# NeLy-EPFL/flygym

Hardware: AMD Instinct MI355X
Metric: env-steps/sec (whole node), 4096 flies per GPU, flat terrain (higher is better)
Workload: dtype f32

## Files before the change

### flygym_amd/csrc/nmf_step.hip

```cpp
#include "nmf_device.h"
#include "nmf_step_lds.h"
#include "nmf_step_diag.h"
#include "nmf_step_kinematics.h"
#include "nmf_step_collision.h"
#include "nmf_step_aba.h"
#include "nmf_step_contact.h"
#include "nmf_dual.h"
#include "nmf_step_noslip.h"
#include "nmf_step_actuation.h"
#include "nmf_step_forward.h"
#include "nmf_step_io.h"
#include "nmf_tree.h"

namespace nmf {

template <class TP> constexpr int waves_per_simd() { return 2; }

template <class TP>
__device__ __forceinline__ void stage_launch_constants(FlyLds<TP>& s, const GModel& m) {
  if constexpr (!TP::kStar) { if (threadIdx.x == 0) { s.rt_nb = m.nb; s.rt_nv = m.nv; } __syncthreads(); }
  if constexpr (TP::kNFact > 1) {
    for (int b = threadIdx.x; b < TP::kTblB && b < m.nb; b += kWave) {
      s.t_body[b] = (unsigned char)m.tree_body[b < m.tree_lvl_start[m.tree_nlevel] ? b : 0];
      s.t_parent[b] = (unsigned char)(b ? m.body_parent[b] : 0);
      s.t_dofadr[b] = (unsigned char)m.body_dofadr[b]; s.t_dofnum[b] = (unsigned char)m.body_dofnum[b];
      s.t_cstart[b] = (unsigned char)m.tree_child_start[b]; s.t_ccount[b] = (unsigned char)m.tree_child_count[b];
    }
    for (int j = threadIdx.x; j < TP::kTblV && j < m.nv; j += kWave) s.t_dofbody[j] = (unsigned char)m.dof_body[j];
    if (threadIdx.x < 18) s.t_lvl[threadIdx.x] = (unsigned char)m.tree_lvl_start[threadIdx.x];
    if (threadIdx.x == 0) s.t_nlevel = (unsigned char)m.tree_nlevel;
    if constexpr (TP::kStar) {
      for (int i = threadIdx.x; i < kRestLevels * 16; i += kWave) (&s.t_pack[0][0][0])[i] = m.rest_fast ? m.rest_pack[i] : 0xffffffffu;
    }
    __syncthreads();
  }
  const int lane = threadIdx.x;
  for (int j = lane; j < s.nv(); j += kWave) {
    if constexpr (row_width_s<TP>() > 6) s.S[j][6] = 0.f;
    s.arm[j] = m.dof_armature[j];
    if constexpr (kHasCm3<TP>) { s.damp[j] = m.dof_damping[j]; s.dlt[j] = m.dof_armature[j] + m.timestep * m.dof_damping[j]; }
  }
  if (lane < 6) {
    const KLane K = k_lane(lane, make_frame(v3(m.plane[0], m.plane[1], m.plane[2])));
    float* q = s.k_tab[lane];
#pragma unroll
    for (int i = 0; i < 3; ++i) { q[i] = K.dA[i]; q[3 + i] = K.dB[i]; q[6 + i] = K.dO[i]; }
    q[9] = __int_as_float(K.ia); q[10] = __int_as_float(K.ib);
    int words[3];
    inertia_map_pack(lane, words);
    q[11] = __int_as_float(words[0]); q[12] = __int_as_float(words[1]); q[13] = __int_as_float(words[2]);
    if constexpr (kHasIsym<TP>) {
#pragma unroll
      for (int c = 0; c < 6; c++) {
        const int i = lane < c ? lane : c, jx = lane < c ? c : lane;
        q[14 + c] = __int_as_float(i * 6 - i * (i - 1) / 2 + (jx - i));
      }
    }
  }
  if constexpr (kHasIsym<TP>) if (lane == 0) {
    const Frame fr = make_frame(v3(m.plane[0], m.plane[1], m.plane[2]));
    st3(&s.frame9[0], fr.n); st3(&s.frame9[3], fr.t1); st3(&s.frame9[6], fr.t2);
    HotModel& h = s.hot;
    h.dof_axis = m.dof_axis; h.body_pos = m.body_pos; h.body_quat = m.body_quat; h.geom_p0 = m.geom_p0; h.geom_p1 = m.geom_p1;
    h.geom_radius = m.geom_radius; h.geom_bsphere = m.geom_bsphere; h.hull_vert = m.hull_vert; h.pair_margin = m.pair_margin;
    h.geom_body = m.geom_body; h.geom_type = m.geom_type; h.geom_hulladr = m.geom_hulladr; h.geom_hullnum = m.geom_hullnum;
#pragma unroll
    for (int i = 0; i < 4; ++i) h.plane[i] = m.plane[i];
#pragma unroll
    for (int i = 0; i < 5; ++i) h.terrain[i] = m.terrain[i];
    h.hull_skin = m.hull_skin; h.terrain_type = m.terrain_type; h.ng = m.ng; h.sem_max_hull_contacts = m.sem_max_hull_contacts;
    h.terrain_walls = m.sem_terrain_walls;
  }
  if constexpr (kHasIsym<TP>) for (int i = lane; i < 3 * s.nv(); i += kWave) (&s.axis[0][0])[i] = m.dof_axis[i];
}

template <class TP>
__global__ void __launch_bounds__(kWave) nmf_reset_kernel(const DevModel* __restrict__ mp, DevState st, const unsigned char* __restrict__ reset_mask) {
  __shared__ FlyLds<TP> s;
  const GModel& m = *(const GModel*)mp;
  const int lane = threadIdx.x, w = (int)blockIdx.x;
  if (w >= st.n_worlds || (reset_mask && !reset_mask[w])) return;
  stage_launch_constants(s, m);
  for (int i = lane; i < s.nq(); i += kWave) s.qpos[i] = m.key_qpos[i];
  for (int i = lane; i < s.nv(); i += kWave) { s.qvel[i] = 0.f; s.qacc[i] = 0.f; }
  for (int i = lane; i < m.nu; i += kWave) { s.ctrl[i] = m.key_ctrl[i]; st.actuator_force[(size_t)w * m.nu + i] = 0.f; st.act[(size_t)w * m.nu + i] = 0.f; }
  for (int i = lane; i < 96; i += kWave) st.sensordata[(size_t)w * 96 + i] = 0.f;
  if (lane == 0) { s.ncon = 0; s.iters = 0; s.overflow = 0; s.solve_resid = 0.f; }
  WSYNC();
  stage_kinematics(s, m, lane);
  write_poses(s, m, st, w, lane);
  write_outputs(s, m, st, w, lane, 0.f, true);
  if (lane < 16) st.stats_sum[16 * (size_t)w + lane] = 0u;
  if (lane < kActHistWords) st.act_hist[(size_t)w * kActHistWords + lane] = 0u;
  if (lane < kMaxCon) st.contact_geom[(size_t)w * kMaxCon + lane] = -1.f;
}

template <class TP, bool WELD>
__global__ void __launch_bounds__(kWave) __attribute__((amdgpu_waves_per_eu(waves_per_simd<TP>(), waves_per_simd<TP>()))) nmf_step_kernel(const DevModel* __restrict__ mp, DevState st, ReplayArgs rp, int n_steps) {
  __shared__ FlyLds<TP> s;
  const GModel& m = *(const GModel*)mp;
  const unsigned long long probe_c0 = __builtin_amdgcn_s_memtime(), probe_r0 = __builtin_amdgcn_s_memrealtime();
  TRACE_DECL();
  const int lane = threadIdx.x;
  const bool chunked = st.sched_mode == 1;
  unsigned int t_first = 0;
  if (chunked && lane == 0) t_first = atomicAdd(&st.csched->ticket, 1u);
  stage_launch_constants(s, m);
  if constexpr (kDualGlob<TP>) { if (lane == 0) s.dual_glob[0] = st.dual_scratch + (size_t)blockIdx.x * kDualScratchFloats; }
  if constexpr (kEulerFused<TP>) {
    if (lane == 0) {
      const unsigned long long p = (unsigned long long)(st.dual_scratch + (size_t)blockIdx.x * euler_scratch_floats<TP>());
      s.euler_fac[0] = (unsigned int)p; s.euler_fac[1] = (unsigned int)(p >> 32);
    }
  }
  unsigned int t_next = (unsigned int)__builtin_amdgcn_readfirstlane((int)t_first);
  STAGE_INIT();
  const int n_chunks = chunked ? st.n_chunks : 1;
  const unsigned int epoch = chunked ? (unsigned int)__builtin_amdgcn_readfirstlane((int)st.csched->epoch) : 0u;
  for (;;) {
    int slot = (int)blockIdx.x, chunk = 0, step0 = 0, step1 = n_steps;
    if (chunked) {
      const unsigned int t = t_next;
      if (t >= (unsigned int)st.n_worlds * (unsigned int)n_chunks) {
        if (lane == 0 && atomicAdd(&st.csched->exited, 1u) == gridDim.x - 1u) {
          st.csched->ticket = 0u; st.csched->exited = 0u; st.csched->epoch = epoch + 1u;
        }
        break;
      }
      chunk = (int)(t / (unsigned int)st.n_worlds); slot = (int)(t % (unsigned int)st.n_worlds);
      step0 = st.chunk_start[chunk]; step1 = st.chunk_start[chunk + 1];
    } else if (slot >= st.n_worlds) return;
    const int w = __builtin_amdgcn_readfirstlane(st.order ? st.order[slot] : slot);
    TRACE_SUB(2);
    const unsigned long long t_begin = __builtin_amdgcn_s_memtime();
    if (st.sched && lane == 0) atomicMin(&st.sched->t_first, (unsigned long long)__builtin_amdgcn_s_memrealtime());
    float time;
    unsigned int carry = 0u;
    unsigned int sum_con = 0u, sum_it = 0u, sum_of = 0u;
    unsigned int sum_dual = 0u, sum_kkt = 0u;
    {
      const float* tab = rp.table ? rp.table + (size_t)w * rp.table_steps * rp.n_act : nullptr;
      const int ln = opaque(lane);
      const int my_ctrl = tab && lane < rp.n_act ? rp.act_ids[ln] : -1;
      CtrlPrefetch pf;
      pf.mine = my_ctrl >= 0; pf.next_row = nullptr;
      pf.value = my_ctrl >= 0 ? tab[(size_t)((rp.start + step0) % rp.table_steps) * rp.n_act + lane] : 0.f;
      if (chunk > 0) {
        const unsigned int want = (unsigned int)__builtin_amdgcn_readfirstlane((int)(epoch * 32u + (unsigned int)chunk));
        const unsigned long long* hb = st.handoff + (size_t)w * st.handoff_stride;
        const int nq = s.nq(), nv = s.nv();
        for (;;) {
          bool ok = true;
          for (int i = ln; i < nq; i += kWave) s.qpos[i] = ld_tagged(&hb[i], want, ok);
          for (int i = ln; i < nv; i += kWave) { s.qvel[i] = ld_tagged(&hb[nq + i], want, ok); s.qacc[i] = ld_tagged(&hb[nq + nv + i], want, ok); }
          for (int i = ln; i < m.nu; i += kWave) s.ctrl[i] = ld_tagged(&hb[nq + 2 * nv + i], want, ok);
          carry = lane < 6 ? ld_tagged_u(&hb[nq + 2 * nv + m.nu + ln], want, ok) : 0u;
          if constexpr (kDual<TP>) { const unsigned int hw = lane < hist_words<TP>(m) ? ld_tagged_u(&hb[nq + 2 * nv + m.nu + 6 + ln], want, ok) : 0u; if (lane < kHistLds<TP>) s.act_hist[lane] = hw; }
          if (!__any(!ok)) break;
          __builtin_amdgcn_s_sleep(8);
        }
        time = __uint_as_float((unsigned int)__builtin_amdgcn_readlane((int)carry, 0));
      } else {
        for (int i = ln; i < s.nq(); i += kWave) s.qpos[i] = ld_state(&st.qpos[(size_t)w * s.nq() + i]);
        for (int i = ln; i < s.nv(); i += kWave) {
          s.qvel[i] = ld_state(&st.qvel[(size_t)w * s.nv() + i]);
          s.qacc[i] = ld_state(&st.qacc_ws[(size_t)w * s.nv() + i]);
        }
        for (int i = ln; i < m.nu; i += kWave) s.ctrl[i] = ld_state(&st.ctrl[(size_t)w * m.nu + i]);
        if constexpr (kDual<TP>) { if (lane < kHistLds<TP>) s.act_hist[lane] = st.act_hist[(size_t)w * kActHistWords + ln]; }
        time = ld_state(&st.time[w]);
      }
      WSYNC();
      TRACE_GAP_END();
      for (int step = step0; step < step1; ++step) {
        if (tab) {
          if (my_ctrl >= 0) s.ctrl[my_ctrl] = pf.value;
          const float* src = tab + (size_t)((rp.start + step) % rp.table_steps) * rp.n_act;
          for (int a = opaque(lane) + kWave; a < rp.n_act; a += kWave) s.ctrl[rp.act_ids[a]] = src[a];
          pf.next_row = step + 1 < step1 ? tab + (size_t)((rp.start + step + 1) % rp.table_steps) * rp.n_act : nullptr;
          WSYNC();
        }
        STAGE(0);
        float* rec = nullptr;
        if (st.obs_every > 0 && (step + 1) % st.obs_every == 0)
          rec = st.ring + ((size_t)((step + 1) / st.obs_every - 1) * (size_t)st.n_worlds + (size_t)w) * (size_t)st.ring_stride;
        const bool wrenches = physics_forward<TP, WELD>(s, m, lane, st, w, step == n_steps - 1, rec, pf STAGE_PASS);
        physics_integrate<TP, WELD>(s, m, lane, wrenches STAGE_PASS);
        if (rec) {
          const int nj = st.ring_nj;
          for (int i = opaque(lane); i < nj; i += kWave) { rec[i] = s.qpos[7 + i]; rec[nj + i] = s.qvel[6 + i]; }
        }
        STAGE(15);
        time += m.timestep;
        const unsigned int rep = (unsigned int)__builtin_amdgcn_readfirstlane(s.iters);
        sum_con += (unsigned int)s.ncon; sum_it += rep & 0xffu; sum_of += (unsigned int)s.overflow;
        sum_dual += (rep >> 8) & 1u; sum_kkt += (rep >> 9) & 1u;
        if (rep & (0xffcu << 8)) {
          const int xl = opaque(lane) - 6;
          if (xl >= 2 && xl < kExitKinds && ((rep >> (8 + xl)) & 1u)) add_count(&st.stats_sum[16 * (size_t)w + 4 + xl], 1u);
        }
      }
    }
    TRACE_BUSY_END();
    TRACE_SUB_RESET();
    unsigned int t_new = 0;
    if (chunked && lane == 0) t_new = atomicAdd(&st.csched->ticket, 1u);
    {
      const unsigned int own = lane == 1 ? (unsigned int)(step1 - step0) : lane == 2 ? sum_con : lane == 3 ? sum_it : sum_of;
      const float cyc = (float)(__builtin_amdgcn_s_memtime() - t_begin);
      if (lane >= 1 && lane <= 4) carry += own;
      if (lane == 5) carry = __float_as_uint(__uint_as_float(carry) + cyc);
      const bool final = step1 == n_steps;
      if (lane == 6 || lane == 7) add_count(&st.stats_sum[16 * (size_t)w + opaque(lane) - 2], lane == 6 ? sum_dual : sum_kkt);
      write_outputs(s, m, st, w, lane, time, final, epoch * 32u + (unsigned int)(chunk + 1), carry);
      if (final) {
        if (lane >= 1 && lane <= 4) add_count(&st.stats_sum[16 * (size_t)w + opaque(lane) - 1], carry);
        if (lane == 5) st_state(&st.cost[w], __uint_as_float(carry));
      }
      if (st.sched && lane == 0) atomicMax(&st.sched->t_last, (unsigned long long)__builtin_amdgcn_s_memrealtime());
    }
    if (!chunked) break;
    TRACE_SUB(0);
    t_next = (unsigned int)__builtin_amdgcn_readfirstlane((int)t_new);
    TRACE_SUB(1);
    WSYNC();
  }
  TRACE_FLUSH();
  if (blockIdx.x == 0 && lane == 0 && st.clock_probe) {
    atomicAdd(&st.clock_probe[0], __builtin_amdgcn_s_memtime() - probe_c0);
    atomicAdd(&st.clock_probe[1], __builtin_amdgcn_s_memrealtime() - probe_r0);
  }
  STAGE(16);
  STAGE_FLUSH();
}

#define NMF_INSTANTIATE(k, TP, ...) NMF_IF_TOPO_##k(                                                      \
  template __global__ void nmf_step_kernel<TP, false>(const DevModel*, DevState, ReplayArgs, int);        \
  template __global__ void nmf_step_kernel<TP, true>(const DevModel*, DevState, ReplayArgs, int);         \
  template __global__ void nmf_step_kernel<Terrain<TP>, false>(const DevModel*, DevState, ReplayArgs, int);)
NMF_FAMILIES(NMF_INSTANTIATE)
#undef NMF_INSTANTIATE

}
```

### flygym_amd/csrc/nmf_step_collision.h

```cpp
#pragma once
#include "nmf_device.h"

namespace nmf {

__device__ __forceinline__ float terrain_kind(int kind, float p0, float p1, float p2, float x, float y) {
  if (kind == 1) { const float period = p0 + p1; const float u = x - floorf(x / period) * period; return u < p0 ? 0.f : -p2; }
  if (kind == 2) { const float i = floorf(x / p0), j = floorf(y / p0); const float sum = i + j;
                   const float par = sum - 2.f * floorf(sum / 2.f); return par != 0.f ? p1 : 0.f; }
  return 0.f;
}
__device__ __forceinline__ float terrain_height(int terrain_type, const float* p, float x, float y) {
  if (terrain_type == 3) {
    const float st = floorf(x / p[3]); const float k = st - 3.f * floorf(st / 3.f);
    return k == 1.f ? terrain_kind(1, 1.0f, p[1], p[2], x, y) : (k == 2.f ? terrain_kind(2, p[0], 0.35f, 0.f, x, y) : 0.f);
  }
  return terrain_kind(terrain_type, p[0], p[1], p[2], x, y);
}

constexpr float kFar = 1e30f;
constexpr float kProbeEps = 1e-4f;
constexpr float kOneCell = 0.02f;
__device__ __forceinline__ float terrain_cell_kind(int kind, float p0, float p1, float p2, float x, float y, float* b) {
  b[0] = -kFar; b[1] = kFar; b[2] = -kFar; b[3] = kFar;
  if (kind == 1) {
    const float period = p0 + p1; const float k = floorf(x / period); const float u = x - k * period;
    if (u < p0) { b[0] = k * period; b[1] = k * period + p0; return 0.f; }
    b[0] = k * period + p0; b[1] = (k + 1.f) * period; return -p2;
  }
  if (kind == 2) {
    const float i = floorf(x / p0), j = floorf(y / p0);
    b[0] = i * p0; b[1] = (i + 1.f) * p0; b[2] = j * p0; b[3] = (j + 1.f) * p0;
    const float sum = i + j; const float par = sum - 2.f * floorf(sum / 2.f);
    return par != 0.f ? p1 : 0.f;
  }
  return 0.f;
}
__device__ __forceinline__ float terrain_cell(int terrain_type, const float* p, float x, float y, float* b) {
  if (terrain_type == 3) {
    const float st = floorf(x / p[3]); const float k = st - 3.f * floorf(st / 3.f);
    const float h = k == 1.f ? terrain_cell_kind(1, 1.0f, p[1], p[2], x, y, b) : (k == 2.f ? terrain_cell_kind(2, p[0], 0.35f, 0.f, x, y, b)
                                                                                            : terrain_cell_kind(0, 0.f, 0.f, 0.f, x, y, b));
    const float lo = st * p[3], hi = (st + 1.f) * p[3];
    if (b[0] < lo) b[0] = lo;
    if (b[1] > hi) b[1] = hi;
    return h;
  }
  return terrain_cell_kind(terrain_type, p[0], p[1], p[2], x, y, b);
}
__device__ __forceinline__ void terrain_probe(int terrain_type, const float* p, bool walls, float x, float y, float zc, float rho,
                                              float reach, float& dtop, float& dwall, int& wall) {
  float b[4];
  const float h0 = terrain_cell(terrain_type, p, x, y, b);
  const float zb = zc - rho;
  dtop = zb - h0; dwall = kFar; wall = 0;
  if (!walls) return;
  const float delta[4] = {b[1] - x, x - b[0], b[3] - y, y - b[2]};
  if (zb >= h0 && fminf(fminf(delta[0], delta[1]), fminf(delta[2], delta[3])) - rho > reach) return;
  const float pen0 = h0 - zb;
  float he[4];
#pragma unroll
  for (int e = 0; e < 4; ++e) {
    he[e] = h0;
    if (delta[e] < kFar && (delta[e] - rho <= reach || (zb < h0 && delta[e] + rho < pen0)))
      he[e] = e == 0 ? terrain_height(terrain_type, p, b[1] + kProbeEps, y) : e == 1 ? terrain_height(terrain_type, p, b[0] - kProbeEps, y)
            : e == 2 ? terrain_height(terrain_type, p, x, b[3] + kProbeEps) : terrain_height(terrain_type, p, x, b[2] - kProbeEps);
  }
  float edge_top = kFar;
#pragma unroll
  for (int e = 0; e < 4; ++e) {
    if (!(delta[e] - rho <= reach && he[e] > zb)) continue;
    if (zc - he[e] > delta[e]) edge_top = fminf(edge_top, zb - he[e]);
    else if (delta[e] - rho < dwall) { dwall = delta[e] - rho; wall = (e ^ 1) + 1; }
  }
  if (zb < h0) {
    float pen = h0 - zb; int code = 0;
#pragma unroll
    for (int e = 0; e < 4; ++e)
      if (delta[e] < kFar && he[e] <= zb && delta[e] + rho < pen) { pen = delta[e] + rho; code = e + 1; }
    if (code) { dtop = kFar; if (-pen < dwall) { dwall = -pen; wall = code; } }
  }
  dtop = fminf(dtop, edge_top);
}

struct CollisionScratch {
  float r[kMaxCon][3], dist[kMaxCon];
  int info[kMaxCon];
};

__device__ __forceinline__ float readlane_f(float v, int lane) {
  return __builtin_bit_cast(float, __builtin_amdgcn_readlane(__builtin_bit_cast(int, v), lane));
}

template <class TP, bool ROUGH>
__device__ __noinline__ void stage_collision(FlyLds<TP>& s, const GModel& m, int lane) {
  static_assert(sizeof(CollisionScratch) <= sizeof(float) * TP::NB * 12, "collision scratch does not fit T..W");
  CollisionScratch& X = *reinterpret_cast<CollisionScratch*>(&s.T[0][0]);
  constexpr bool kSlotInTW = sizeof(CollisionScratch) + 2 * kWave * sizeof(int) <= sizeof(float) * TP::NB * 12;
  static_assert(kSlotInTW || 3 * (TP::NB - 1) + 2 * kWave <= 7 * kMaxCon, "slot table (128 geoms) does not fit");
  int* geom_slot0 = kSlotInTW ? reinterpret_cast<int*>(&s.T[0][0]) + sizeof(CollisionScratch) / sizeof(int)
                              : reinterpret_cast<int*>(&s.c_w[0][0]) + 3 * (TP::NB - 1);
  constexpr int kTwUsed = (int)sizeof(CollisionScratch) + (kSlotInTW ? 2 * kWave * (int)sizeof(int) : 0);
  constexpr int kCandRoom = ((int)sizeof(float) * TP::NB * 12 - kTwUsed) / 8;
  constexpr int kCand = kCandRoom > kWave ? kWave : kCandRoom;
  constexpr bool kListed = ROUGH && kCand >= 8;
  int* cand_idx = reinterpret_cast<int*>(&s.T[0][0]) + kTwUsed / 4;
  float* cand_d = reinterpret_cast<float*>(cand_idx + (kCand > 0 ? kCand : 0));
  const HotModel hm = hot_model(s, m);
  const int ng = hm.ng, terrain_type = hm.terrain_type, max_hull_contacts = hm.sem_max_hull_contacts;
  const bool walls = hm.terrain_walls != 0;
  const float hull_skin = hm.hull_skin, terrain_top = hm.terrain[4];
  const float tpar[4] = {hm.terrain[0], hm.terrain[1], hm.terrain[2], hm.terrain[3]};
  const gptr<int> geom_body = G(hm.geom_body), geom_type = G(hm.geom_type), geom_hulladr = G(hm.geom_hulladr),
                  geom_hullnum = G(hm.geom_hullnum);
  const gptr<float> pair_margin = G(hm.pair_margin), geom_bsphere = G(hm.geom_bsphere), geom_radius = G(hm.geom_radius),
                    geom_p0 = G(hm.geom_p0), geom_p1 = G(hm.geom_p1), hull_vert = G(hm.hull_vert);
  const V3 n = ld3(hm.plane);
  const float pd = hm.plane[3];
  const V3 o = ld3(s.xpos()[0]);
  constexpr bool rough = ROUGH;
  SUB_T0();
  int nh = 0, slot_base = 0;
  for (int g0 = 0; g0 < ng; g0 += kWave) {
  const int gi = g0 + lane;
  int g_body = 0, g_type = -1, g_hadr = 0, g_hnum = 0, cnt = 0;
  float g_margin = 0.f, cd0 = 0.f, cd1 = 0.f;
  V3 cp0 = v3(0, 0, 0), cp1 = v3(0, 0, 0);
  float cdw0 = 0.f, cdw1 = 0.f; V3 cpw0 = v3(0, 0, 0), cpw1 = v3(0, 0, 0); int cfid = 0, cntw = 0;
  bool near = false;
  bool one_cell = false; float g_ttop = 0.f;
  if (gi < ng) {
    g_body = geom_body[gi]; g_type = geom_type[gi]; g_margin = pair_margin[gi];
    g_hadr = geom_hulladr[gi]; g_hnum = geom_hullnum[gi];
    const V3 bs = ld3(geom_bsphere + 4 * gi);
    const float bs_r = geom_bsphere[4 * gi + 3], rad = geom_radius[gi];
    const V3 l0 = ld3(geom_p0 + 3 * gi), l1 = ld3(geom_p1 + 3 * gi);
    const float* R = s.xmat()[g_body];
    const V3 xp = ld3(s.xpos()[g_body]);
    V3 cw = mat_vec(R, bs);
    float dc = dot(n, cw) + dot(n, xp) - pd;
    float ttop = terrain_top;
    const V3 p0 = mat_vec(R, l0) + xp, p1 = mat_vec(R, l1) + xp;
    if (rough && dc - bs_r - terrain_top <= g_margin) {
      const float cx = cw.x + xp.x, cy = cw.y + xp.y, fr = bs_r + g_margin, fc = rad + g_margin;
      const float fx0 = fmaxf(cx - fr, fminf(p0.x, p1.x) - fc), fx1 = fminf(cx + fr, fmaxf(p0.x, p1.x) + fc);
      const float fy0 = fmaxf(cy - fr, fminf(p0.y, p1.y) - fc), fy1 = fminf(cy + fr, fmaxf(p0.y, p1.y) + fc);
      const float mx = 0.5f * (fx0 + fx1), my = 0.5f * (fy0 + fy1);
      float cb[4];
      ttop = terrain_cell(terrain_type, tpar, mx, my, cb);
      const float clear = fminf(fminf(cb[1] - fx1, fx0 - cb[0]), fminf(cb[3] - fy1, fy0 - cb[2]));
      one_cell = clear > kOneCell;
      if (!(clear > 0.f)) {
        if (terrain_type >= 2 && tpar[0] < 0.5f * (fy1 - fy0)) ttop = terrain_top;
        else {
          float xs = fx0;
          bool open = true;
#pragma unroll 1
          for (int k = 0; k < 8 && open; ++k) {
            float wb[4];
            ttop = fmaxf(ttop, terrain_cell(terrain_type, tpar, xs, my, wb));
            ttop = fmaxf(ttop, fmaxf(terrain_height(terrain_type, tpar, xs, fy0), terrain_height(terrain_type, tpar, xs, fy1)));
            open = wb[1] <= fx1;
            xs = wb[1] + kProbeEps;
          }
          if (open) ttop = terrain_top;
        }
      }
      g_ttop = ttop;
    }
    near = dc - bs_r - ttop <= g_margin;
    const float z0 = dot(n, p0) - pd, z1 = dot(n, p1) - pd;
    float d0 = z0 - rad, d1 = z1 - rad;
    if (g_type == GEOM_HULL) {
      const V3 ax = p1 - p0;
      const float ca = dot(n, ax);
      const float sn = sqrtf(fmaxf(0.f, 1.f - ca * ca / fmaxf(dot(ax, ax), 1e-12f)) + 4e-6f);
      near = near && fminf(z0, z1) - rad * fminf(sn, 1.f) - ttop <= g_margin;
    } else if (rough) near = near && fminf(d0, d1) - ttop <= g_margin;
    if (near && g_type == GEOM_CAPSULE) {
      float dw0 = kFar, dw1 = kFar; int w0 = 0, w1 = 0;
      if (rough) {
        if (one_cell && fminf(d0, d1) - g_ttop >= -kOneCell) { d0 -= g_ttop; d1 -= g_ttop; }
        else {
          terrain_probe(terrain_type, tpar, walls, p0.x, p0.y, z0, rad, g_margin, d0, dw0, w0);
          terrain_probe(terrain_type, tpar, walls, p1.x, p1.y, z1, rad, g_margin, d1, dw1, w1);
        }
      }
      const V3 q0 = ((p0 - rad * n) - (0.5f * d0) * n) - o, q1 = ((p1 - rad * n) - (0.5f * d1) * n) - o;
      if (d0 <= g_margin) { cd0 = d0; cp0 = q0; cnt = 1; }
      if (d1 <= g_margin) { if (cnt) { cd1 = d1; cp1 = q1; } else { cd0 = d1; cp0 = q1; } cnt++; }
      if (rough) {
        if (w0 && dw0 <= g_margin) { const V3 nw = contact_frame(w0, Frame{n, n, n}).n; cdw0 = dw0; cpw0 = ((p0 - rad * nw) - (0.5f * dw0) * nw) - o; cfid = w0; cntw = 1; }
        if (w1 && dw1 <= g_margin) { const V3 nw = contact_frame(w1, Frame{n, n, n}).n; const V3 q = ((p1 - rad * nw) - (0.5f * dw1) * nw) - o;
                                     if (cntw) { cdw1 = dw1; cpw1 = q; cfid |= w1 << 3; } else { cdw0 = dw1; cpw0 = q; cfid = w1; } cntw++; }
        cnt += cntw;
      }
    }
  }
  SUB(21);
  unsigned long long hmask = __ballot(near && g_type == GEOM_HULL);
  const unsigned long long one_mask = __ballot(one_cell);
  SUB_COUNT(24, __popcll(hmask));
  while (hmask) {
    SUBH_T0();
    const int g = __ffsll((long long)hmask) - 1;
    hmask &= hmask - 1;
    const int b = __builtin_amdgcn_readlane(g_body, g);
    const float margin = readlane_f(g_margin, g);
    const gptr<float> V = hull_vert + 3 * __builtin_amdgcn_readlane(g_hadr, g);
    const int nvv = __builtin_amdgcn_readlane(g_hnum, g);
    const float* R = s.xmat()[b];
    const V3 xp = ld3(s.xpos()[b]);
    const V3 nb = matT_vec(R, n);
    const float c0 = dot(n, xp) - pd;
    float pdw = kFar; int pw_code = 0;
    bool one = rough && ((one_mask >> g) & 1ull);
    const float h_top = rough ? readlane_f(g_ttop, g) : 0.f;
    auto vdist = [&](V3 v) {
      float di = dot(nb, v) + c0;
      if (rough) {
        pw_code = 0;
        if (one || di - h_top > margin) di = di - h_top;
        else { const V3 pw = mat_vec(R, v) + xp; terrain_probe(terrain_type, tpar, walls, pw.x, pw.y, di, 0.f, margin, di, pdw, pw_code); }
      }
      return di;
    };
    SUBH(28);
    float best = INFINITY; int bi = 0x7fffffff;
    float bestw = INFINITY; int biw = 0x7fffffff;
    int ncand = 0;
    for (;;) {
    best = INFINITY; bi = 0x7fffffff; ncand = 0;
    for (int base = lane; base < nvv + lane; base += 4 * kWave) {
      V3 hv[4];
#pragma unroll
      for (int k = 0; k < 4; ++k) { const int i = base + k * kWave; hv[k] = ld3(V + 3 * (i < nvv ? i : nvv - 1)); }
#pragma unroll
      for (int k = 0; k < 4; ++k) {
        const int i = base + k * kWave;
        bool c = false; float di = 0.f;
        if (i < nvv) {
          di = vdist(hv[k]);
          if (di < best) { best = di; bi = i; }
          if (rough && pw_code && pdw < bestw) { bestw = pdw; biw = i * 8 + pw_code; }
          c = di <= margin;
        }
        if constexpr (kListed) {
          const unsigned long long cm = __ballot(c);
          const int pos = ncand + __popcll(cm & ((1ull << lane) - 1ull));
          if (c && pos < kCand) { cand_idx[pos] = i; cand_d[pos] = di; }
          ncand += __popcll(cm);
        }
      }
    }
    wave_argmin(best, bi);
    if (rough && one && !(best >= -kOneCell)) { one = false; continue; }
    break;
    }
    const float dmin = best; const int ia = bi;
    bool face = false;
    if (rough && walls) { wave_argmin(bestw, biw); face = bestw <= margin; }
    SUBH(29); SUB_COUNT(32, one ? 1 : 0); SUB_COUNT(33, nvv);
    if (!(dmin <= margin) && !face) { SUB_COUNT(25, 1); SUB_COUNT(26, (unsigned long long)(fminf(dmin, 1.f) * 1e6f)); continue; }
    SUB_COUNT(27, 1);
    int nsel = 0;
    int s1 = -1, s2 = -1, s3 = -1;
    [[maybe_unused]] int listed_dbg = 0;
    if (dmin <= margin) {
    nsel = 1;
    const float thr = fminf(dmin + hull_skin, margin);
    const V3 va = ld3(V + 3 * ia);
    bool listed = false;
    if constexpr (kListed) listed = ncand <= kCand;
    listed_dbg = listed ? 1 : 0;
    if (listed) {
      if constexpr (kListed) {
        WSYNC();
        const bool have = lane < ncand;
        const int ci = have ? cand_idx[lane] : 0;
        const bool ok = have && !(cand_d[have ? lane : 0] > thr);
        const V3 vi = ld3(V + 3 * ci);
        auto pick = [&](int idx) {
          const int wl = __ffsll((long long)__ballot(ok && ci == idx)) - 1;
          return v3(readlane_f(vi.x, wl), readlane_f(vi.y, wl), readlane_f(vi.z, wl));
        };
        { const V3 e = vi - va; best = ok ? dot(e, e) : -INFINITY; bi = ok ? ci : 0x7fffffff; }
        wave_argmax(best, bi);
        if (best > 1e-10f) {
          s1 = bi; nsel = 2;
          const V3 ab = pick(bi) - va;
          const float lab2 = dot(ab, ab);
          { const V3 cr = cross(vi - va, ab); best = ok ? dot(cr, cr) : -INFINITY; bi = ok ? ci : 0x7fffffff; }
          wave_argmax(best, bi);
          if (best > 1e-10f * lab2) {
            s2 = bi; nsel = 3;
            const float side = dot(cross(pick(bi) - va, ab), nb);
            const float sg = side > 0.f ? -1.f : 1.f;
            best = ok ? sg * dot(cross(vi - va, ab), nb) : -INFINITY; bi = ok ? ci : 0x7fffffff;
            wave_argmax(best, bi);
            if (best > sqrtf(1e-10f * lab2)) { s3 = bi; nsel = 4; }
          }
        }
        WSYNC();
      }
    } else {
    best = -INFINITY; bi = 0x7fffffff;
    for (int i = lane; i < nvv; i += kWave) {
      V3 vi = ld3(V + 3 * i);
      float di = vdist(vi);
      if (di > thr) continue;
      V3 e = vi - va; float sc = dot(e, e);
      if (sc > best) { best = sc; bi = i; }
    }
    wave_argmax(best, bi);
    if (best > 1e-10f) {
      s1 = bi; nsel = 2;
      const V3 ab = ld3(V + 3 * bi) - va;
      const float lab2 = dot(ab, ab);
      best = -INFINITY; bi = 0x7fffffff;
      for (int i = lane; i < nvv; i += kWave) {
        V3 vi = ld3(V + 3 * i);
        float di = vdist(vi);
        if (di > thr) continue;
        V3 cr = cross(vi - va, ab); float sc = dot(cr, cr);
        if (sc > best) { best = sc; bi = i; }
      }
      wave_argmax(best, bi);
      if (best > 1e-10f * lab2) {
        s2 = bi; nsel = 3;
        const float side = dot(cross(ld3(V + 3 * bi) - va, ab), nb);
        const float sg = side > 0.f ? -1.f : 1.f;
        best = -INFINITY; bi = 0x7fffffff;
        for (int i = lane; i < nvv; i += kWave) {
          V3 vi = ld3(V + 3 * i);
          float di = vdist(vi);
          if (di > thr) continue;
          float sc = sg * dot(cross(vi - va, ab), nb);
          if (sc > best) { best = sc; bi = i; }
        }
        wave_argmax(best, bi);
        if (best > sqrtf(1e-10f * lab2)) { s3 = bi; nsel = 4; }
      }
    }
    }
    nsel = nsel < max_hull_contacts ? nsel : max_hull_contacts;
    }
    SUBH(30); SUB_COUNT(34, listed_dbg);
    if (lane < nsel && nh + lane < kMaxCon) {
      const int vi = lane == 0 ? ia : lane == 1 ? s1 : lane == 2 ? s2 : s3;
      const V3 v = ld3(V + 3 * vi);
      float dist = lane == 0 ? dmin : vdist(v);
      if (rough && lane != 0 && !(dist <= margin)) dist = fminf(dmin + hull_skin, margin);
      const V3 pw = mat_vec(R, v) + xp;
      X.info[nh + lane] = (g0 + g) | (lane << 8) | (b << 12);
      X.dist[nh + lane] = dist;
      st3(X.r[nh + lane], (pw - (0.5f * dist) * n) - o);
    }
    if (face && lane == nsel && nh + lane < kMaxCon) {
      const int code = biw & 7;
      const V3 nw = contact_frame(code, Frame{n, n, n}).n;
      const V3 pw = mat_vec(R, ld3(V + 3 * (biw >> 3))) + xp;
      X.info[nh + lane] = (g0 + g) | (lane << 8) | (b << 12) | (code << 20);
      X.dist[nh + lane] = bestw;
      st3(X.r[nh + lane], (pw - (0.5f * bestw) * nw) - o);
    }
    nsel += face ? 1 : 0;
    if (lane == g) cnt = nsel;
    nh += nsel;
    SUBH(31);
  }
  SUB(22);
  const unsigned long long b0 = __ballot(cnt & 1), b1 = __ballot(cnt & 2), b2 = __ballot(cnt & 4);
  const unsigned long long lt = (1ull << lane) - 1ull;
  const int slot0 = __popcll(b0 & lt) + 2 * __popcll(b1 & lt) + 4 * __popcll(b2 & lt);
  const int sl = slot_base + slot0;
  geom_slot0[gi] = slot_base + slot0;
  if (g_type == GEOM_CAPSULE && cnt > 0) {
    const int ntop = cnt - cntw;
    if (ntop > 0 && sl < kMaxCon) { s.c_info[sl] = info_pack(gi, -1, g_body, 0); s.c_D[sl] = cd0; st3(s.c_r[sl], cp0); }
    if (ntop > 1 && sl + 1 < kMaxCon) { s.c_info[sl + 1] = info_pack(gi, -1, g_body, 0); s.c_D[sl + 1] = cd1; st3(s.c_r[sl + 1], cp1); }
    if (cntw > 0 && sl + ntop < kMaxCon) { s.c_info[sl + ntop] = info_pack(gi, -1, g_body, 0) | ((cfid & 7) << 24); s.c_D[sl + ntop] = cdw0; st3(s.c_r[sl + ntop], cpw0); }
    if (cntw > 1 && sl + ntop + 1 < kMaxCon) { s.c_info[sl + ntop + 1] = info_pack(gi, -1, g_body, 0) | ((cfid >> 3) << 24); s.c_D[sl + ntop + 1] = cdw1; st3(s.c_r[sl + ntop + 1], cpw1); }
  }
  slot_base += __popcll(b0) + 2 * __popcll(b1) + 4 * __popcll(b2);
  }
  const int total = slot_base;
  WSYNC();
  if (lane < nh && lane < kMaxCon) {
    const int info = X.info[lane];
    const int slot = geom_slot0[info & 0xff] + ((info >> 8) & 0xf);
    if (slot < kMaxCon) { s.c_info[slot] = info_pack(info & 0xff, -1, (info >> 12) & 0xff, 0) | (((info >> 20) & 7) << 24); s.c_D[slot] = X.dist[lane]; st3(s.c_r[slot], ld3(X.r[lane])); }
  }
  const int cap = m.max_contacts;
  const int ncon = total > cap ? cap : total;
  if (lane == 0) { s.ncon = ncon; s.overflow = total > cap ? 1 : 0; }
  WSYNC();
  {
    if constexpr (rough) {
      const unsigned long long wf = __ballot(lane < ncon && info_fid(s.c_info[lane]) != 0);
      if (lane == 0) s.nwall = __popcll(wf);
    }
  }
  bool ranged = false;
  if constexpr (TP::kStar) { if constexpr (TP::NB + 1 <= kWave) {
    ranged = true;
    const int e = lane < ncon ? info_body(s.c_info[lane]) : 0x7fffffff;
    const int e_prev = lane > 0 && lane - 1 < ncon ? info_body(s.c_info[lane > 0 ? lane - 1 : 0]) : -1;
    if (lane <= TP::NB) s.body_cstart[lane] = (typename FlyLds<TP>::cstart_t)ncon;
    WSYNC();
    if (lane < ncon && e != e_prev) s.body_cstart[e] = (typename FlyLds<TP>::cstart_t)lane;
    WSYNC();
    const int b = kWave - 1 - lane;
    const int first = wave_prefix_min_int(b <= TP::NB ? (int)s.body_cstart[b <= TP::NB ? b : 0] : 0x7fffffff);
    WSYNC();
    if (b <= TP::NB) s.body_cstart[b] = (typename FlyLds<TP>::cstart_t)first;
  } }
// ... 13 lines not shown
```

### flygym_amd/csrc/nmf_step_io.h

```cpp
#pragma once
#include "nmf_device.h"

namespace nmf {

__device__ __forceinline__ float ld_state(const float* p) { return __hip_atomic_load(p, __ATOMIC_RELAXED, __HIP_MEMORY_SCOPE_AGENT); }
__device__ __forceinline__ void st_state(float* p, float v) { __hip_atomic_store(p, v, __ATOMIC_RELAXED, __HIP_MEMORY_SCOPE_AGENT); }
__device__ __forceinline__ void add_state(float* p, float v) { (void)__hip_atomic_fetch_add(p, v, __ATOMIC_RELAXED, __HIP_MEMORY_SCOPE_AGENT); }
__device__ __forceinline__ void add_count(unsigned int* p, unsigned int v) { (void)__hip_atomic_fetch_add(p, v, __ATOMIC_RELAXED, __HIP_MEMORY_SCOPE_AGENT); }

__device__ __forceinline__ void st_tagged(unsigned long long* p, float v, unsigned int tag) {
  __hip_atomic_store(p, ((unsigned long long)tag << 32) | (unsigned long long)__float_as_uint(v), __ATOMIC_RELAXED, __HIP_MEMORY_SCOPE_AGENT);
}
__device__ __forceinline__ float ld_tagged(const unsigned long long* p, unsigned int want, bool& ok) {
  const unsigned long long g = __hip_atomic_load(p, __ATOMIC_RELAXED, __HIP_MEMORY_SCOPE_AGENT);
  ok = ok && (unsigned int)(g >> 32) == want;
  return __uint_as_float((unsigned int)g);
}
__device__ __forceinline__ void st_tagged_u(unsigned long long* p, unsigned int v, unsigned int tag) {
  __hip_atomic_store(p, ((unsigned long long)tag << 32) | (unsigned long long)v, __ATOMIC_RELAXED, __HIP_MEMORY_SCOPE_AGENT);
}
__device__ __forceinline__ unsigned int ld_tagged_u(const unsigned long long* p, unsigned int want, bool& ok) {
  const unsigned long long g = __hip_atomic_load(p, __ATOMIC_RELAXED, __HIP_MEMORY_SCOPE_AGENT);
  ok = ok && (unsigned int)(g >> 32) == want;
  return (unsigned int)g;
}

template <class TP>
__device__ void write_outputs(FlyLds<TP>& s, const GModel& m, const DevState& st, int w, int lane, float time, bool final,
                              unsigned int tag = 0u, unsigned int carry = 0u) {
  lane = opaque(lane);
  if (!final) {
    unsigned long long* hb = st.handoff + (size_t)w * st.handoff_stride;
    const int nq = s.nq(), nv = s.nv();
    for (int i = lane; i < nq; i += kWave) st_tagged(&hb[i], s.qpos[i], tag);
    for (int i = lane; i < nv; i += kWave) { st_tagged(&hb[nq + i], s.qvel[i], tag); st_tagged(&hb[nq + nv + i], s.qacc[i], tag); }
    for (int i = lane; i < m.nu; i += kWave) st_tagged(&hb[nq + 2 * nv + i], s.ctrl[i], tag);
    if (lane < 6) st_tagged_u(&hb[nq + 2 * nv + m.nu + lane], lane == 0 ? __float_as_uint(time) : carry, tag);
    if constexpr (kDual<TP>) { if (lane < hist_words<TP>(m)) st_tagged_u(&hb[nq + 2 * nv + m.nu + 6 + lane], s.act_hist[lane], tag); }
    return;
  }
  if constexpr (kDual<TP>) { if (lane < kActHistWords) st.act_hist[(size_t)w * kActHistWords + lane] = lane < hist_words<TP>(m) ? s.act_hist[lane < kHistLds<TP> ? lane : 0] : 0u; }
  const bool noslip_qacc = m.noslip_iter > 0 && st.noslip_buf && s.ncon > 0 && ((unsigned int)s.iters & (kExitPrimal | kExitDual)) != 0u;
  for (int i = lane; i < s.nq(); i += kWave) st_state(&st.qpos[(size_t)w * s.nq() + i], s.qpos[i]);
  for (int i = lane; i < s.nv(); i += kWave) {
    st_state(&st.qvel[(size_t)w * s.nv() + i], s.qvel[i]);
    st_state(&st.qacc_ws[(size_t)w * s.nv() + i], s.qacc[i]);
    if (final && !noslip_qacc) st.qacc[(size_t)w * s.nv() + i] = s.qacc[i];
  }
  for (int i = lane; i < m.nu; i += kWave) {
    st_state(&st.ctrl[(size_t)w * m.nu + i], s.ctrl[i]);
  }
  if (lane == 0) st_state(&st.time[opaque(w)], time);
  if (lane == 0 && final) {
    float* q = &st.stats[8 * (size_t)w];
    q[0] = (float)s.ncon; q[1] = (float)(s.iters & 0xff); q[2] = (float)s.overflow; q[3] = (float)(4 * s.ncon);
    q[4] = (float)((s.iters >> 8) & 0xfff); q[5] = (float)((s.iters >> 20) & 0x7f); q[6] = s.solve_resid; q[7] = 0.f;
  }
}

template <class TP>
__device__ void write_poses(FlyLds<TP>& s, const GModel& m, const DevState& st, int w, int lane) {
  lane = opaque(lane);
  for (int sg = lane; sg < m.nseg; sg += kWave) {
    int b = m.seg_body[sg];
    V3 p = ld3(s.xpos()[b]) + mat_vec(s.xmat()[b], ld3(&m.seg_pos[3 * sg]));
    Q4 q = qnorm(qmul(mat_quat(s.xmat()[b]), ldq(&m.seg_quat[4 * sg])));
    if (q.w < 0.f) q = Q4{-q.w, -q.x, -q.y, -q.z};
    st3(&st.seg_xpos[((size_t)w * m.nseg + sg) * 3], p);
    stq(&st.seg_xquat[((size_t)w * m.nseg + sg) * 4], q);
  }
  for (int sg = lane; sg < m.nsite; sg += kWave) {
    int b = m.site_body[sg];
    V3 p = ld3(s.xpos()[b]) + mat_vec(s.xmat()[b], ld3(&m.site_pos[3 * sg]));
    st3(&st.site_xpos[((size_t)w * m.nsite + sg) * 3], p);
  }
}

}
```

### flygym_amd/csrc/nmf_step_lds.h

```cpp
#pragma once
#include "nmf_device.h"

namespace nmf {

#define WSYNC() do { __builtin_amdgcn_fence(__ATOMIC_SEQ_CST, "wavefront"); __builtin_amdgcn_wave_barrier(); } while (0)
constexpr float kNoiseFactor = 8.f;
enum : unsigned int {
  kExitDual = 1u << 8,
  kExitKkt = 1u << 9,
  kExitTie = 1u << 10,
  kExitStall = 1u << 11,
  kExitCost = 1u << 12,
  kExitMaxIter = 1u << 13,
  kExitPrimal = 1u << 14,
  kExitFallback = 1u << 15,
  kExitBigPivots = 1u << 16,
  kExitNoNoslip = 1u << 17,
  kExitFree = 1u << 18,
};
constexpr int kExitKinds = 12;
constexpr int kDualRegPivots = 47;
constexpr float kDualResidMax = 1e-3f;
constexpr int kDualExitFrom = 5;

#define NMF_TREE_TABLES                                                                                                  \
  unsigned char t_body[TP::kTblB], t_parent[TP::kTblB], t_dofadr[TP::kTblB], t_dofnum[TP::kTblB], t_cstart[TP::kTblB],    \
      t_ccount[TP::kTblB], t_dofbody[TP::kTblV];                                                                          \
  unsigned char t_lvl[18], t_nlevel;

template <class TP, bool STAR = TP::kStar, bool REST = (TP::kNFact > 1)>
struct TreeLds {};
template <class TP>
struct TreeLds<TP, false, true> {
  float fact[TP::kNFact][8];
  float slot[TP::kNSlot][27];
  int rt_nb, rt_nv;
  NMF_TREE_TABLES
};
template <class TP>
struct TreeLds<TP, true, true> {
  float fact[TP::kNFact][8];
  int reduced;
  float restA[21];
  unsigned int t_pack[kRestLevels][8][2];
  NMF_TREE_TABLES
};

template <class TP> constexpr bool has_cm3() { if constexpr (TP::kStar) return TP::REST_B == 0; else return false; }
template <class TP> inline constexpr bool kHasCm3 = has_cm3<TP>();
template <class TP> inline constexpr bool kHasIsym = has_cm3<TP>();

constexpr bool rows_conflict_free(int rows_per_leg, int width, int nleg) {
  const int ng = nleg < 4 ? nleg : 4;
  for (int a = 0; a < ng; ++a)
    for (int b = a + 1; b < ng; ++b) {
      const int d = (((b - a) * rows_per_leg * width) % 32 + 32) % 32;
      if (d < 6 || d > 26) return false;
    }
  return true;
}
constexpr int conflict_free_width(int rows_per_leg, int nleg) {
  for (int w = 6; w <= 9; ++w) if (rows_conflict_free(rows_per_leg, w, nleg)) return w;
  return 6;
}
template <class TP> constexpr int row_width_s() { if constexpr (TP::kStar) return TP::REST_B == 0 ? conflict_free_width(TP::NDL, TP::NLEG) : 6; else return 6; }
template <class TP> constexpr int row_width_tw() { if constexpr (TP::kStar) return TP::REST_B == 0 ? conflict_free_width(TP::NBL, TP::NLEG) : 6; else return 6; }
template <class TP> constexpr bool dual_hybrid() {
  if constexpr (TP::kStar) return TP::REST_B > 0; else return false;
}
template <class TP> constexpr bool dual_global() {
  if constexpr (TP::kStar) return TP::REST_B > 0 && 4 * TP::NV < TP::NLEG * TP::NDL * 8; else return false;
}
template <class TP> inline constexpr bool kDualS = has_cm3<TP>();
template <class TP> inline constexpr bool kDualH = dual_hybrid<TP>();
template <class TP> inline constexpr bool kDual = kDualS<TP> || kDualH<TP>;
template <class TP> inline constexpr bool kDualGlob = kDualH<TP> && dual_global<TP>();
constexpr int kDualScratchFloats = 8 * 6 * 24;
template <class TP> constexpr bool euler_fused() {
#ifdef NMF_EULER_REFACTOR
  return false;
#else
  return has_cm3<TP>();
#endif
}
template <class TP> inline constexpr bool kEulerFused = euler_fused<TP>();
template <class TP> constexpr int euler_scratch_floats() { if constexpr (has_cm3<TP>()) return 8 * (TP::NLEG * TP::NDL + 6); else return 0; }
constexpr int dual_g_floats(int ncon) { return 9 * ncon * (ncon + 1) / 2; }
template <class TP> constexpr int dual_max_con() {
  if constexpr (kDualH<TP>) {
    int n = 0;
    while (n < 16 && dual_g_floats(n + 1) <= 2 * TP::NB * 6) ++n;
    return n;
  } else return 16;
}
template <class TP> inline constexpr int kDualMaxCon = dual_max_con<TP>();
template <class TP> inline constexpr int kHistLds = kDualS<TP> ? kActHistWords : kDualH<TP> ? 5 : 0;
template <class TP, class M> __device__ __forceinline__ int hist_words(const M& m) {
  if constexpr (kDualS<TP>) return (m.ng + 1) / 2; else return kHistLds<TP>;
}
template <class TP> constexpr int dual_pad_floats() {
  if constexpr (kDualS<TP>) {
    constexpr int need = dual_g_floats(kDualMaxCon<TP>);
    constexpr int have = TP::NB * 11 + 2 * TP::NB * (TP::REST_B == 0 ? conflict_free_width(TP::NBL, TP::NLEG) : 6);
    return need > have ? need - have : 0;
  } else return 0;
}

struct HotModel {
  const float *dof_axis, *body_pos, *body_quat, *geom_p0, *geom_p1, *geom_radius, *geom_bsphere, *hull_vert, *pair_margin;
  const int *geom_body, *geom_type, *geom_hulladr, *geom_hullnum;
  float plane[4], terrain[5], hull_skin;
  int terrain_type, ng, sem_max_hull_contacts, terrain_walls;
};
template <class TP> struct FlyLds;
template <class TP> struct AbaHandoff;
template <class T> using gptr = const __attribute__((address_space(1))) T*;
template <class T> __device__ __forceinline__ gptr<T> G(const T* p) { return (gptr<T>)p; }
__device__ __forceinline__ V3 ld3(gptr<float> p) { return V3{p[0], p[1], p[2]}; }
__device__ __forceinline__ Q4 ldq(gptr<float> p) { return Q4{p[0], p[1], p[2], p[3]}; }

template <class TP>
struct __align__(16) FlyLds : TreeLds<TP> {
  __device__ __forceinline__ int nv() const { if constexpr (TP::kStar) return TP::NV; else return this->rt_nv; }
  __device__ __forceinline__ int nb() const { if constexpr (TP::kStar) return TP::NB; else return this->rt_nb; }
  __device__ __forceinline__ int nq() const { return nv() + 1; }
  float qpos[TP::NQ + 3];
  float qvel[TP::NV], qacc[TP::NV];
  float xmat_root[9];
  float qacc_smooth[TP::NV], qfrc_smooth[TP::NV];
  float vA[TP::NV], vB[TP::NV], vC[TP::NV], vD[TP::NV];
  float ctrl[TP::kCtrl];
  float S[TP::NV][row_width_s<TP>()];
  float Isym[kHasIsym<TP> ? TP::NB : 1][kHasIsym<TP> ? 21 : 1];
  unsigned int euler_fac[kEulerFused<TP> ? 2 : 0];
  alignas(kDualS<TP> ? 16 : 4) float Ib[TP::NB][kHasCm3<TP> ? 11 : 10];
  static_assert(6 * TP::NV >= 9 * (TP::NB - 1), "rotation matrices do not fit the solver vectors");
  static_assert(7 * kMaxCon >= 3 * (TP::NB - 1), "body positions do not fit the contact wrenches");
  __device__ __forceinline__ float (*xmat())[9] { return reinterpret_cast<float(*)[9]>(&xmat_root[0]); }
  __device__ __forceinline__ const float (*xmat() const)[9] { return reinterpret_cast<const float(*)[9]>(&xmat_root[0]); }
  __device__ __forceinline__ float (*xpos())[3] { return reinterpret_cast<float(*)[3]>(&xpos_root[0]); }
  __device__ __forceinline__ const float (*xpos() const)[3] { return reinterpret_cast<const float(*)[3]>(&xpos_root[0]); }
  float T[TP::NB][row_width_tw<TP>()], W[TP::NB][row_width_tw<TP>()];
  float dual_pad[dual_pad_floats<TP>()];
  float arm[TP::NV], damp[kHasCm3<TP> ? TP::NV : 1];
  float dlt[kHasCm3<TP> ? TP::NV : 1];
  float c_r[kMaxCon][3], c_D[kMaxCon], c_mu[kMaxCon];
  int c_info[kMaxCon];
  alignas(kDualS<TP> ? 16 : 4) float xpos_pad_[kDualS<TP> ? 1 : 0];
  float xpos_root[3];
  float c_w[kMaxCon][7];
  float c_m3[kHasCm3<TP> ? kMaxCon : 1][kHasCm3<TP> ? 5 : 1];
  float k_tab[6][kHasIsym<TP> ? 20 : 14];
  float frame9[kHasIsym<TP> ? 9 : 1];
  std::conditional_t<kHasIsym<TP>, HotModel, char> hot;
  float axis[kHasIsym<TP> ? TP::NV : 1][3];
  float weldD[6], weld_w[6];
  using cstart_t = std::conditional_t<kHasIsym<TP>, int, unsigned char>;
  cstart_t body_cstart[(TP::NB + 1 + 3) / 4 * 4];
  __device__ __forceinline__ float* slot_at(int k) {
    if constexpr (TP::kStar) {
      constexpr int kInCw = 7 * kMaxCon / 27;
      static_assert(TP::REST_B == 0 || (TP::REST_B - kInCw) * 27 * sizeof(float) + sizeof(AbaHandoff<TP>) <= sizeof(float) * TP::NB * 2 * row_width_tw<TP>(),
                    "hand-off slots of the rest do not fit T..W");
      return k < kInCw ? &c_w[0][0] + 27 * k : &T[0][0] + sizeof(AbaHandoff<TP>) / sizeof(float) + 27 * (k - kInCw);
    } else return this->slot[k];
  }
  unsigned int act_hist[kHistLds<TP>];
  float* dual_glob[kDualGlob<TP> ? 1 : 0];
  int ncon, overflow;
  int iters;
  float solve_resid;
  int nwall;
  __device__ __forceinline__ float* vec(int id) {
    switch (id) {
      case 0: return qacc;
      case 1: return qacc_smooth;
      case 2: return qfrc_smooth;
      case 3: return vA;
      case 4: return vB;
      case 5: return vC;
      default: return vD;
    }
  }
};
template <class TP> __device__ __forceinline__ HotModel hot_model(const FlyLds<TP>& s, const GModel& m) {
  if constexpr (kHasIsym<TP>) return s.hot;
  else {
    HotModel h;
    h.dof_axis = (const float*)m.dof_axis; h.body_pos = (const float*)m.body_pos; h.body_quat = (const float*)m.body_quat;
    h.geom_p0 = (const float*)m.geom_p0; h.geom_p1 = (const float*)m.geom_p1; h.geom_radius = (const float*)m.geom_radius;
    h.geom_bsphere = (const float*)m.geom_bsphere; h.hull_vert = (const float*)m.hull_vert; h.pair_margin = (const float*)m.pair_margin;
    h.geom_body = (const int*)m.geom_body; h.geom_type = (const int*)m.geom_type; h.geom_hulladr = (const int*)m.geom_hulladr;
    h.geom_hullnum = (const int*)m.geom_hullnum;
#pragma unroll
    for (int i = 0; i < 4; ++i) h.plane[i] = m.plane[i];
#pragma unroll
    for (int i = 0; i < 5; ++i) h.terrain[i] = m.terrain[i];
    h.hull_skin = m.hull_skin; h.terrain_type = m.terrain_type; h.ng = m.ng; h.sem_max_hull_contacts = m.sem_max_hull_contacts;
    h.terrain_walls = m.sem_terrain_walls;
    return h;
  }
}
template <class TP> __device__ __forceinline__ float dof_damp(const FlyLds<TP>& s, const GModel& m, int j) {
  if constexpr (kHasCm3<TP>) return s.damp[j]; else return m.dof_damping[j];
}
template <class TP> __device__ __forceinline__ float dof_delta(const FlyLds<TP>& s, const GModel& m, int j, float hdamp) {
  if constexpr (kHasCm3<TP>) return (hdamp != 0.f ? s.dlt : s.arm)[j];
  else return hdamp != 0.f ? fmaf(hdamp, m.dof_damping[j], s.arm[j]) : s.arm[j];
}
template <class TP> __device__ __forceinline__ int tbl_dofbody(const FlyLds<TP>& s, int j) { if constexpr (TP::kNFact > 1) return s.t_dofbody[j]; else return 0; }
template <class TP> __device__ __forceinline__ int tbl_dofadr(const FlyLds<TP>& s, int b) { if constexpr (TP::kNFact > 1) return s.t_dofadr[b]; else return 0; }
template <class TP> __device__ __forceinline__ int tbl_dofnum(const FlyLds<TP>& s, int b) { if constexpr (TP::kNFact > 1) return s.t_dofnum[b]; else return 0; }
enum { V_QACC = 0, V_QACC_SMOOTH = 1, V_QFRC_SMOOTH = 2, V_A = 3, V_B = 4, V_C = 5, V_D = 6 };

__device__ __forceinline__ int info_geom(int i) { return i & 0xff; }
__device__ __forceinline__ int info_sensor(int i) { return ((i >> 8) & 0xf) - 1; }
__device__ __forceinline__ int info_body(int i) { return (i >> 12) & 0xff; }
__device__ __forceinline__ int info_act(int i) { return (i >> 20) & 0xf; }
__device__ __forceinline__ int info_fid(int i) { return (i >> 24) & 0x7; }
__device__ __forceinline__ int info_pack(int geom, int sensor, int body, int act) {
  return geom | ((sensor + 1) << 8) | (body << 12) | (act << 20);
}

template <class TP>
struct AbaHandoff {
  float legIA[TP::NLEG][6][6], legpA[TP::NLEG][6], rootA[6][6], rootb[6];
};

struct Frame { V3 n, t1, t2; };

template <class LDS> __device__ __forceinline__ Frame ld_frame(const LDS& s, const GModel& m);
__device__ __forceinline__ Frame make_frame(V3 n) {
  V3 t = fabsf(n.y) < 0.5f ? v3(0.f, 1.f, 0.f) : v3(0.f, 0.f, 1.f);
  float dn = dot(t, n);
  V3 t1 = t - dn * n;
  float l = sqrtf(dot(t1, t1));
  t1 = (1.0f / l) * t1;
  return Frame{n, t1, cross(n, t1)};
}

template <class LDS> __device__ __forceinline__ Frame ld_frame(const LDS& s, const GModel& m) {
  if constexpr (sizeof(s.frame9) == 9 * sizeof(float)) return Frame{ld3(&s.frame9[0]), ld3(&s.frame9[3]), ld3(&s.frame9[6])};
  else return make_frame(v3(m.plane[0], m.plane[1], m.plane[2]));
}

__device__ __forceinline__ Frame contact_frame(int fid, const Frame& f0) {
  const float sg = (fid & 1) ? 1.f : -1.f;
  const bool xw = fid <= 2, pl = fid == 0;
  Frame f;
  f.n = pl ? f0.n : (xw ? v3(sg, 0.f, 0.f) : v3(0.f, sg, 0.f));
  f.t1 = pl ? f0.t1 : (xw ? v3(0.f, 1.f, 0.f) : v3(0.f, 0.f, 1.f));
  f.t2 = pl ? f0.t2 : (xw ? v3(0.f, 0.f, sg) : v3(sg, 0.f, 0.f));
  return f;
}

template <class TP>
__device__ __forceinline__ int dof_body_of(int j) {
  if (j < 6) return 0;
  const int leg = (j - TP::LD0) / TP::NDL, d = (j - TP::LD0) % TP::NDL;
  int lb = 0;
  static_for<TP::NBL - 1>([&](auto I) { constexpr int l = decltype(I)::value; lb += d >= TP::first_dof(l + 1) ? 1 : 0; });
  return TP::LB0 + leg * TP::NBL + lb;
}

struct LaneRole {
  int grp, r, lg, rr;
  bool live;
  float mask;
};
template <class TP>
__device__ __forceinline__ LaneRole lane_role(int lane) {
  LaneRole L;
  L.grp = lane >> 3; L.r = lane & 7;
  L.lg = L.grp < TP::NLEG ? L.grp : TP::NLEG - 1;
  L.rr = L.r < 6 ? L.r : 5;
  L.live = L.grp < TP::NLEG && L.r < 6;
  L.mask = L.r < 6 ? 1.f : 0.f;
  return L;
}

}
```

Measured before the change: 64.23 million.

## Skip hull-plane vertex scans using cached separation bounds from earlier steps

Adds a small per-fly LDS cache of hull-vs-plane scan results. When a hull was proven far from the plane, the cache keeps its minimum distance and the body-frame plane normal. Later steps then prove clearance from the rotation change, using a float rounding guard, and skip the full vertex scan. Only flat terrain uses it. This adds LDS state, an extra ballot branch in the broadphase and conservative-bound logic that must stay correct as poses change. An optional tally counter for skip statistics is also added.

```diff
diff --git a/flygym_amd/csrc/nmf_scan_bound.h b/flygym_amd/csrc/nmf_scan_bound.h
--- /dev/null
+++ b/flygym_amd/csrc/nmf_scan_bound.h
@@ -0,0 +1,30 @@
+#pragma once
+#if !defined(__HIPCC__)
+#include <cmath>
+#endif
+
+namespace nmf {
+
+#if defined(__HIPCC__)
+#define NMF_BOUND_FN __device__ __forceinline__
+#else
+#define NMF_BOUND_FN inline
+#endif
+
+constexpr int kScanRefSlots = 6;
+constexpr float kScanGuardRel = 1.f / 262144.f;
+
+struct ScanRef { int tag; float nb[3]; float e; };
+
+NMF_BOUND_FN float scan_guard(float nx, float ny, float nz, float px, float py, float pz, float pd, float bx, float by, float bz, float r) {
+  return kScanGuardRel * (fabsf(nx * px) + fabsf(ny * py) + fabsf(nz * pz) + fabsf(pd) + fabsf(bx) + fabsf(by) + fabsf(bz) + r);
+}
+NMF_BOUND_FN float scan_ref_value(float dmin, float dc, float guard) { return (dmin - dc) - guard; }
+NMF_BOUND_FN bool scan_proved_clear(float e_ref, float rx, float ry, float rz, float nbx, float nby, float nbz, float dc, float r,
+                                    float guard, float margin) {
+  const float dx = nbx - rx, dy = nby - ry, dz = nbz - rz;
+  const float L = (e_ref + dc) - sqrtf(dx * dx + dy * dy + dz * dz) * r;
+  return L - guard > margin;
+}
+
+}
diff --git a/flygym_amd/csrc/nmf_step.hip b/flygym_amd/csrc/nmf_step.hip
--- a/flygym_amd/csrc/nmf_step.hip
+++ b/flygym_amd/csrc/nmf_step.hip
@@ -72,6 +72,7 @@
     h.terrain_walls = m.sem_terrain_walls;
   }
   if constexpr (kHasIsym<TP>) for (int i = lane; i < 3 * s.nv(); i += kWave) (&s.axis[0][0])[i] = m.dof_axis[i];
+  if constexpr (kScanSkip<TP>) { if (lane < kScanRefSlots) s.scan_ref[lane].tag = -1; }
 }
 
 template <class TP>
@@ -93,6 +94,7 @@
   if (lane < 16) st.stats_sum[16 * (size_t)w + lane] = 0u;
   if (lane < kActHistWords) st.act_hist[(size_t)w * kActHistWords + lane] = 0u;
   if (lane < kMaxCon) st.contact_geom[(size_t)w * kMaxCon + lane] = -1.f;
+  if constexpr (kScanTally<TP>) { if (lane == 0) st.stats[8 * (size_t)w + 7] = 0.f; }
 }
 
 template <class TP, bool WELD>
@@ -170,6 +172,7 @@
         if constexpr (kDual<TP>) { if (lane < kHistLds<TP>) s.act_hist[lane] = st.act_hist[(size_t)w * kActHistWords + ln]; }
         time = ld_state(&st.time[w]);
       }
+      if constexpr (kScanTally<TP>) { if (lane == 0) s.scan_tally[0] = 0u; }
       WSYNC();
       TRACE_GAP_END();
       for (int step = step0; step < step1; ++step) {
@@ -213,6 +216,7 @@
       const bool final = step1 == n_steps;
       if (lane == 6 || lane == 7) add_count(&st.stats_sum[16 * (size_t)w + opaque(lane) - 2], lane == 6 ? sum_dual : sum_kkt);
       write_outputs(s, m, st, w, lane, time, final, epoch * 32u + (unsigned int)(chunk + 1), carry);
+      if constexpr (kScanTally<TP>) { if (lane == 0) add_count(reinterpret_cast<unsigned int*>(&st.stats[8 * (size_t)w + 7]), s.scan_tally[0]); }
       if (final) {
         if (lane >= 1 && lane <= 4) add_count(&st.stats_sum[16 * (size_t)w + opaque(lane) - 1], carry);
         if (lane == 5) st_state(&st.cost[w], __uint_as_float(carry));
diff --git a/flygym_amd/csrc/nmf_step_collision.h b/flygym_amd/csrc/nmf_step_collision.h
--- a/flygym_amd/csrc/nmf_step_collision.h
+++ b/flygym_amd/csrc/nmf_step_collision.h
@@ -118,6 +118,7 @@
   const float pd = hm.plane[3];
   const V3 o = ld3(s.xpos()[0]);
   constexpr bool rough = ROUGH;
+  constexpr bool kSkip = kScanSkip<TP> && !ROUGH;
   SUB_T0();
   int nh = 0, slot_base = 0;
   for (int g0 = 0; g0 < ng; g0 += kWave) {
@@ -176,6 +177,22 @@
       const float sn = sqrtf(fmaxf(0.f, 1.f - ca * ca / fmaxf(dot(ax, ax), 1e-12f)) + 4e-6f);
       near = near && fminf(z0, z1) - rad * fminf(sn, 1.f) - ttop <= g_margin;
     } else if (rough) near = near && fminf(d0, d1) - ttop <= g_margin;
+    if constexpr (kSkip) {
+      const bool hull_near = near && g_type == GEOM_HULL;
+      if (__any(hull_near)) {
+        bool clear = false;
+        if (hull_near) {
+          const V3 nb = matT_vec(R, n);
+          const ScanRef& ref = s.scan_ref[gi % kScanRefSlots];
+          const float guard = scan_guard(n.x, n.y, n.z, xp.x, xp.y, xp.z, pd, bs.x, bs.y, bs.z, bs_r);
+          clear = ref.tag == gi && scan_proved_clear(ref.e, ref.nb[0], ref.nb[1], ref.nb[2], nb.x, nb.y, nb.z, dc, bs_r, guard, g_margin);
+          near = !clear;
+        }
+        [[maybe_unused]] const int nclear = __popcll(__ballot(clear));
+        SUB_COUNT(35, nclear);
+        if constexpr (kScanTally<TP>) { if (lane == 0) s.scan_tally[0] += (unsigned int)nclear << 16; }
+      }
+    }
     if (near && g_type == GEOM_CAPSULE) {
       float dw0 = kFar, dw1 = kFar; int w0 = 0, w1 = 0;
       if (rough) {
@@ -212,6 +229,8 @@
     const V3 xp = ld3(s.xpos()[b]);
     const V3 nb = matT_vec(R, n);
     const float c0 = dot(n, xp) - pd;
+    [[maybe_unused]] V3 ref_bs = v3(0, 0, 0); [[maybe_unused]] float ref_r = 0.f;
+    if constexpr (kSkip) { ref_bs = ld3(geom_bsphere + 4 * (g0 + g)); ref_r = geom_bsphere[4 * (g0 + g) + 3]; }
     float pdw = kFar; int pw_code = 0;
     bool one = rough && ((one_mask >> g) & 1ull);
     const float h_top = rough ? readlane_f(g_ttop, g) : 0.f;
@@ -260,7 +279,19 @@
     bool face = false;
     if (rough && walls) { wave_argmin(bestw, biw); face = bestw <= margin; }
     SUBH(29); SUB_COUNT(32, one ? 1 : 0); SUB_COUNT(33, nvv);
-    if (!(dmin <= margin) && !face) { SUB_COUNT(25, 1); SUB_COUNT(26, (unsigned long long)(fminf(dmin, 1.f) * 1e6f)); continue; }
+    if constexpr (kScanTally<TP>) { if (lane == 0) s.scan_tally[0] += 1u; }
+    if (!(dmin <= margin) && !face) {
+      SUB_COUNT(25, 1); SUB_COUNT(26, (unsigned long long)(fminf(dmin, 1.f) * 1e6f));
+      if constexpr (kSkip) {
+        const float guard = scan_guard(n.x, n.y, n.z, xp.x, xp.y, xp.z, pd, ref_bs.x, ref_bs.y, ref_bs.z, ref_r);
+        if (lane == 0) {
+          ScanRef& ref = s.scan_ref[(g0 + g) % kScanRefSlots];
+          ref.tag = g0 + g; ref.nb[0] = nb.x; ref.nb[1] = nb.y; ref.nb[2] = nb.z;
+          ref.e = scan_ref_value(dmin, dot(nb, ref_bs) + c0, guard);
+        }
+      }
+      continue;
+    }
     SUB_COUNT(27, 1);
     int nsel = 0;
     int s1 = -1, s2 = -1, s3 = -1;
diff --git a/flygym_amd/csrc/nmf_step_io.h b/flygym_amd/csrc/nmf_step_io.h
--- a/flygym_amd/csrc/nmf_step_io.h
+++ b/flygym_amd/csrc/nmf_step_io.h
@@ -54,7 +54,8 @@
   if (lane == 0 && final) {
     float* q = &st.stats[8 * (size_t)w];
     q[0] = (float)s.ncon; q[1] = (float)(s.iters & 0xff); q[2] = (float)s.overflow; q[3] = (float)(4 * s.ncon);
-    q[4] = (float)((s.iters >> 8) & 0xfff); q[5] = (float)((s.iters >> 20) & 0x7f); q[6] = s.solve_resid; q[7] = 0.f;
+    q[4] = (float)((s.iters >> 8) & 0xfff); q[5] = (float)((s.iters >> 20) & 0x7f); q[6] = s.solve_resid;
+    if constexpr (!kScanTally<TP>) q[7] = 0.f;
   }
 }
 
diff --git a/flygym_amd/csrc/nmf_step_lds.h b/flygym_amd/csrc/nmf_step_lds.h
--- a/flygym_amd/csrc/nmf_step_lds.h
+++ b/flygym_amd/csrc/nmf_step_lds.h
@@ -1,5 +1,6 @@
 #pragma once
 #include "nmf_device.h"
+#include "nmf_scan_bound.h"
 
 namespace nmf {
 
@@ -84,6 +85,19 @@
 #endif
 }
 template <class TP> inline constexpr bool kEulerFused = euler_fused<TP>();
+template <class TP> constexpr bool scan_skip() {
+#ifdef NMF_NO_SCAN_SKIP
+  return false;
+#else
+  return has_cm3<TP>() && !TP::kTerrain;
+#endif
+}
+template <class TP> inline constexpr bool kScanSkip = scan_skip<TP>();
+#ifdef NMF_SCAN_TALLY
+template <class TP> inline constexpr bool kScanTally = has_cm3<TP>() && !TP::kTerrain;
+#else
+template <class TP> inline constexpr bool kScanTally = false;
+#endif
 template <class TP> constexpr int euler_scratch_floats() { if constexpr (has_cm3<TP>()) return 8 * (TP::NLEG * TP::NDL + 6); else return 0; }
 constexpr int dual_g_floats(int ncon) { return 9 * ncon * (ncon + 1) / 2; }
 template <class TP> constexpr int dual_max_con() {
@@ -171,6 +185,8 @@
   int iters;
   float solve_resid;
   int nwall;
+  ScanRef scan_ref[kScanSkip<TP> ? kScanRefSlots : 0];
+  unsigned int scan_tally[kScanTally<TP> ? 1 : 0];
   __device__ __forceinline__ float* vec(int id) {
     switch (id) {
       case 0: return qacc;
```

Result: no change. 64.69 million (median of 6 runs) (+0.7%).
